# rcallahan/smalt

Hardware: AMD Instinct MI355X
Metric: mapped reads/sec (1Mx150bp vs 3Gbp ref) (higher is better)
Workload: dtype f16

## Files before the change

### smalt_amd/csrc/smg_kernels.hip

```cpp
#include <hip/hip_runtime.h>
#include <cstdlib>
#include "smg_kernels.h"
#include "smg_stages.hpp"

namespace smg {

__device__ inline uint8_t code_of(uint8_t c) {
  c &= 0xDF;
  return c == 'A' ? 0 : c == 'C' ? 1 : c == 'G' ? 2 : (c == 'T' || c == 'U') ? 3 : 5;
}

__global__ void __launch_bounds__(64) k_encode(const uint8_t *bases, const uint64_t *off, uint32_t n, uint8_t *codes, uint8_t *codes_rc) {
  for (uint32_t r = blockIdx.x; r < n; r += gridDim.x) {
    const uint64_t o = off[r];
    const uint32_t len = (uint32_t)(off[r + 1] - o);
    for (uint32_t i = threadIdx.x; i < len; i += 64) {
      uint8_t c = code_of(bases[o + i]);
      codes[o + i] = c;
      codes_rc[o + len - 1 - i] = (c & 4) ? c : (uint8_t)(3 - c);
    }
  }
}

__global__ void __launch_bounds__(64) k_gather_reads(uint8_t *dst_bases, uint8_t *dst_quals, const uint64_t *dst_off, uint32_t n, const uint32_t *ids,
// ... 171 lines not shown
  __shared__ uint32_t qslot;
  uint32_t *cursor = b.next_item + NEXT_ITEM_STRIDE * (pass == 2 ? 3 : 2);
  if (pass == 2) {
    const uint32_t n = *b.align_retry_n;
    for (uint32_t i = next_item(cursor, &qslot); i < n; i = next_item(cursor, &qslot)) {
      stage_align<WIDE>(b, ix, p, b.align_retry[i], x);
      __syncthreads();
    }
    align_tally_flush(b, x);
    return;
  }
  for (uint32_t r = next_item(cursor, &qslot); r < b.nreads; r = next_item(cursor, &qslot)) {
    stage_align<WIDE>(b, ix, p, r, x);
    __syncthreads();
  }
  align_tally_flush(b, x);
}

template <int G>
__device__ inline int shr1(int v) {
  return __builtin_amdgcn_update_dpp(0, v, 0x111 , 0xf, 0xf, true);
}

template <int G, int C>
__global__ void __launch_bounds__(64) k_sw_full(Batch b, DevIndex ix, MapPar p, uint32_t ntask_cap, int after16) {
  if (after16 && b.work[WK_QN_TASKS] == 0) return;
  constexpr int NG = 64 / G;
  constexpr int WMAX = SW_FULL_WMAX;
  __shared__ uint8_t win[NG][WMAX + 8];
  __shared__ uint2 tab[8];
  const int lane = threadIdx.x, g = lane % G, grp = lane / G;
  const uint32_t ntask = min(*b.rc_count, ntask_cap);
  const int bias = (p.mismatch < p.mismatch - p.match ? -p.mismatch : -(p.mismatch - p.match));
  const int gi = -p.gap_init, ge = -p.gap_ext;
  if (lane < 8) {
    int rb = lane == 7 ? 0 : ((lane == 6 || lane == 4) ? 5 : lane);
    uint32_t w[2] = {0, 0};
    for (int qc = 0; qc < 8; qc++) {
      int v = (rb == 5 || qc >= 4) ? 0 : ((rb == qc) ? p.match : p.mismatch);
      w[qc >> 2] |= (uint32_t)((v + bias) & 0xff) << (8 * (qc & 3));
    }
    tab[lane] = make_uint2(w[0], w[1]);
  }
  __syncthreads();
  const uint32_t ngroups = gridDim.x * NG;
  unsigned long long cells = 0, ntasks_done = 0;
  for (uint32_t t0 = blockIdx.x * NG; t0 < ntask; t0 += ngroups) {
    const uint32_t t = t0 + grp;
    RCand c;
    bool live = false;
    uint32_t qlen = 0, wlen = 0;
    uint64_t gbase = 0;
    if (t < ntask) {
      c = b.rcpool[t];
      qlen = read_len(b, c.rid);
      wlen = (uint32_t)(c.re - c.rs + 1);
      live = !(c.flags & (RCF_BANDED | RCF_ERR | RCF_SCORED)) && wlen <= (uint32_t)WMAX && qlen <= (uint32_t)(G * C);
      gbase = (c.sqidx < 0 ? 0ull : ix.sop[c.sqidx]) + c.rs;
    }
    if (!live) { qlen = 0; wlen = 0; }
    for (uint32_t i = g; i < wlen; i += G) win[grp][i] = (uint8_t)ref_code(ix.packed, gbase + i);
    uint32_t sel[C];
    {
      const uint8_t *q = ((c.flags & RCF_REVERSE) ? b.codes_rc : b.codes) + (live ? b.read_off[c.rid] : 0);
#pragma unroll
      for (int cc = 0; cc < C; cc++) {
        uint32_t j = (uint32_t)(g * C + cc);
        uint32_t qc = (live && j < qlen) ? q[j] : 5u;
        sel[cc] = 0x0c0c0c00u | qc;
      }
    }
    int H[C], E[C];
#pragma unroll
    for (int cc = 0; cc < C; cc++) { H[cc] = 0; E[cc] = 0; }
    int best = 0, F = 0, prev_hl = 0;
    int nstep = (int)wlen + G - 1;
    for (int o = 32; o > 0; o >>= 1) nstep = max(nstep, __shfl_xor(nstep, o));
    __syncthreads();
    for (int step = 0; step < nstep; step++) {
      const int row = step - g;
      const uint32_t rb = (row >= 0 && row < (int)wlen) ? win[grp][row] : 5u;
      const uint2 tr = tab[rb];
      int hl = shr1<G>(H[C - 1]);
      int fin = shr1<G>(F);
      if (g == 0) { hl = 0; fin = 0; }
      int diag = prev_hl;
      prev_hl = hl;
      F = fin;
#pragma unroll
      for (int cc = 0; cc < C; cc++) {
        const int w = (int)__builtin_amdgcn_perm(tr.y, tr.x, sel[cc]);
        const int h = diag + w - bias;
        const int hh = max(max(h, E[cc]), F);
        best = max(best, hh);
        diag = H[cc];
        H[cc] = hh;
        const int tt = hh - gi;
        E[cc] = max(max(E[cc] - ge, tt), 0);
        F = max(max(F - ge, tt), 0);
      }
    }
    for (int o = G / 2; o > 0; o >>= 1) best = max(best, __shfl_xor(best, o));
    if (live && g == 0) {
      b.rcpool[t].swscor = best;
      b.rcpool[t].flags = c.flags | RCF_SCORED | (best >= 65535 ? RCF_BANDED : 0u);
      cells += (unsigned long long)qlen * wlen;
      ntasks_done += best < 65535 ? 1 : 0;
    }
    __syncthreads();
  }
  for (int o = 32; o > 0; o >>= 1) { cells += __shfl_xor(cells, o); ntasks_done += __shfl_xor(ntasks_done, o); }
  if (lane == 0 && cells) { atomicAdd(b.work + WK_CELLS_FULL, cells); atomicAdd(b.work + WK_TASKS_FULL, ntasks_done); }
}

typedef unsigned short us2 __attribute__((ext_vector_type(2)));
__device__ inline us2 as_us2(uint32_t v) { return __builtin_bit_cast(us2, v); }
__device__ inline uint32_t as_u32(us2 v) { return __builtin_bit_cast(uint32_t, v); }
__device__ inline us2 pk_max(us2 a, us2 b) { return __builtin_elementwise_max(a, b); }
__device__ inline us2 pk_subs(us2 a, us2 b) { return __builtin_elementwise_sub_sat(a, b); }
__device__ inline us2 pk_add_nc(us2 a, us2 b) { return as_us2(as_u32(a) + as_u32(b)); }
typedef _Float16 hf2 __attribute__((ext_vector_type(2)));
__device__ inline us2 pk_max3(us2 a, us2 b, us2 c) {
  const hf2 r = __builtin_elementwise_maximum(__builtin_elementwise_maximum(__builtin_bit_cast(hf2, a), __builtin_bit_cast(hf2, b)), __builtin_bit_cast(hf2, c));
  return __builtin_bit_cast(us2, r);
}
__device__ inline uint32_t shr1_u32(uint32_t v) { return (uint32_t)__builtin_amdgcn_update_dpp(0, (int)v, 0x111 , 0xf, 0xf, true); }

enum : int { SW16_BLK = 5 };
struct Sw16Par { uint32_t mm4, dlt, n4; us2 bias, gi, ge; int fp; uint32_t hi_match, hi_mismatch; us2 ngi, nge; };
__device__ inline uint32_t f16_bits_of_int(int n) {
  if (n == 0) return 0;
  const uint32_t sign = n < 0 ? 0x8000u : 0u, a = (uint32_t)(n < 0 ? -n : n);
  const int e = 31 - __clz((int)a);
  return sign | ((uint32_t)(e + 15) << 10) | ((e <= 10 ? a << (10 - e) : a >> (e - 10)) & 0x3ffu);
}
__device__ inline Sw16Par sw16_par(const MapPar &p, int ncols = 512) {
  Sw16Par s;
  const uint32_t fm = f16_bits_of_int(p.match), fx = f16_bits_of_int(p.mismatch);
  s.fp = (fm & 0xffu) == 0 && (fx & 0xffu) == 0 && p.match > 0 && p.match * ncols <= 2040 && -p.gap_init >= 0 && -p.gap_init <= 2040 &&
         -p.gap_ext >= 0 && -p.gap_ext <= 2040 && p.mismatch >= -1024;
  s.hi_match = fm >> 8; s.hi_mismatch = fx >> 8;
  { const uint32_t a = f16_bits_of_int(p.gap_init), e = f16_bits_of_int(p.gap_ext);
    s.ngi = us2{(unsigned short)a, (unsigned short)a}; s.nge = us2{(unsigned short)e, (unsigned short)e}; }
  const int bias = (p.mismatch < p.mismatch - p.match ? -p.mismatch : -(p.mismatch - p.match));
  s.mm4 = (uint32_t)((p.mismatch + bias) & 0xff) * 0x01010101u;
  s.dlt = (uint32_t)(p.match - p.mismatch);
  s.n4 = (uint32_t)(bias & 0xff) * 0x01010101u;
  s.bias = us2{(unsigned short)bias, (unsigned short)bias};
  s.gi = us2{(unsigned short)(-p.gap_init), (unsigned short)(-p.gap_init)};
  s.ge = us2{(unsigned short)(-p.gap_ext), (unsigned short)(-p.gap_ext)};
  return s;
}

template <int G, int C>
__device__ inline uint32_t sw16_core(const uint16_t *wrow, int nstep, const uint32_t (&sel)[C], int g, const Sw16Par &sp, const uint2 *rowtab2) {
  us2 H[C], E[C];
#pragma unroll
  for (int cc = 0; cc < C; cc++) { H[cc] = us2{0, 0}; E[cc] = us2{0, 0}; }
  us2 best = us2{0, 0}, F = us2{0, 0}, prev_hl = us2{0, 0};
  const uint32_t gmask = g == 0 ? 0u : 0xffffffffu;
  for (int step = 0; step < nstep; step++) {
    const uint2 rr = rowtab2[wrow[step - g + (G - 1)]];
    const uint32_t rowA = rr.x, rowB = rr.y;
    const uint32_t hl = shr1_u32(as_u32(H[C - 1])) & gmask;
    const uint32_t fin = shr1_u32(as_u32(F)) & gmask;
    us2 carry = prev_hl;
    prev_hl = as_us2(hl);
    F = as_us2(fin);
#pragma unroll
    for (int c0 = 0; c0 < C; c0 += SW16_BLK) {
      us2 t3[SW16_BLK];
      const us2 last_old = H[(c0 + SW16_BLK - 1 < C) ? c0 + SW16_BLK - 1 : C - 1];
#pragma unroll
      for (int u = 0; u < SW16_BLK; u++) {
        const int cc = c0 + u;
        if (cc < C) {
          const us2 w = as_us2(__builtin_amdgcn_perm(rowB, rowA, sel[cc]));
          const us2 dg = u == 0 ? carry : H[cc - 1];
          t3[u] = pk_subs(pk_add_nc(dg, w), sp.bias);
        }
      }
#pragma unroll
      for (int u = 0; u < SW16_BLK; u++) {
        const int cc = c0 + u;
        if (cc < C) {
          const us2 hh = pk_max3(t3[u], E[cc], F);
          H[cc] = hh;
          const us2 tt = pk_subs(hh, sp.gi);
          E[cc] = pk_max(pk_subs(E[cc], sp.ge), tt);
          F = pk_max(pk_subs(F, sp.ge), tt);
        }
      }
#pragma unroll
      for (int u = 0; u < SW16_BLK; u += 2) {
        const int cc = c0 + u;
        if (cc + 1 < C && u + 1 < SW16_BLK) best = pk_max3(best, H[cc], H[cc + 1]);
        else if (cc < C) best = pk_max(best, H[cc]);
      }
      carry = last_old;
    }
  }
  uint32_t bb = as_u32(best);
  for (int o = G / 2; o > 0; o >>= 1) bb = as_u32(pk_max(as_us2(bb), as_us2((uint32_t)__shfl_xor((int)bb, o))));
  return bb;
}

__device__ inline hf2 hf_max3(hf2 a, hf2 b, hf2 c) { return __builtin_elementwise_maximum(__builtin_elementwise_maximum(a, b), c); }
template <int G, int C>
__device__ inline uint32_t sw16f_core(const uint16_t *wrow, int nstep, const uint32_t (&sel)[C], int g, const Sw16Par &sp, const uint2 *rowtab2) {
  hf2 H[C], E[C];
  const hf2 zero = hf2{(_Float16)0, (_Float16)0};
#pragma unroll
  for (int cc = 0; cc < C; cc++) { H[cc] = zero; E[cc] = zero; }
  hf2 best = zero, F = zero, prev_hl = zero;
  const hf2 ngi = __builtin_bit_cast(hf2, sp.ngi), nge = __builtin_bit_cast(hf2, sp.nge);
  const uint32_t gmask = g == 0 ? 0u : 0xffffffffu;
  for (int step = 0; step < nstep; step++) {
    const uint2 rr = rowtab2[wrow[step - g + (G - 1)]];
    const uint32_t hl = shr1_u32(__builtin_bit_cast(uint32_t, H[C - 1])) & gmask;
    const uint32_t fin = shr1_u32(__builtin_bit_cast(uint32_t, F)) & gmask;
    hf2 carry = prev_hl;
    prev_hl = __builtin_bit_cast(hf2, hl);
    F = __builtin_bit_cast(hf2, fin);
#pragma unroll
    for (int c0 = 0; c0 < C; c0 += SW16_BLK) {
      hf2 t3[SW16_BLK];
      const hf2 last_old = H[(c0 + SW16_BLK - 1 < C) ? c0 + SW16_BLK - 1 : C - 1];
#pragma unroll
      for (int u = 0; u < SW16_BLK; u++) {
        const int cc = c0 + u;
        if (cc < C) {
          const hf2 w = __builtin_bit_cast(hf2, __builtin_amdgcn_perm(rr.y, rr.x, sel[cc]));
          const hf2 dg = u == 0 ? carry : H[cc - 1];
          t3[u] = dg + w;
        }
      }
#pragma unroll
      for (int u = 0; u < SW16_BLK; u++) {
        const int cc = c0 + u;
        if (cc < C) {
          const hf2 hh = hf_max3(t3[u], E[cc], F);
          H[cc] = hh;
          const hf2 tt = hh + ngi;
          E[cc] = hf_max3(E[cc] + nge, tt, zero);
          F = hf_max3(F + nge, tt, zero);
        }
      }
#pragma unroll
      for (int u = 0; u < SW16_BLK; u += 2) {
        const int cc = c0 + u;
        if (cc + 1 < C && u + 1 < SW16_BLK) best = hf_max3(best, H[cc], H[cc + 1]);
        else if (cc < C) best = __builtin_elementwise_maximum(best, H[cc]);
      }
      carry = last_old;
    }
  }
  for (int o = G / 2; o > 0; o >>= 1)
    best = __builtin_elementwise_maximum(best, __builtin_bit_cast(hf2, (uint32_t)__shfl_xor((int)__builtin_bit_cast(uint32_t, best), o)));
  return (uint32_t)(int)(float)best.x | ((uint32_t)(int)(float)best.y << 16);
}

__device__ inline void sw16_rowtab(uint32_t *rowtab, const Sw16Par &sp) {
  if (threadIdx.x < 8) rowtab[threadIdx.x] = threadIdx.x < 4 ? sp.mm4 + (sp.dlt << (8 * threadIdx.x)) : sp.n4;
}
__device__ inline void sw16_rowtab2(uint2 *rowtab2, const Sw16Par &sp) {
  const uint32_t a = threadIdx.x & 7u, bq = threadIdx.x >> 3;
  if (sp.fp) {
    const uint32_t x4 = sp.hi_mismatch * 0x01010101u;
    rowtab2[threadIdx.x] = make_uint2(a < 4 ? (x4 & ~(0xffu << (8 * a))) | (sp.hi_match << (8 * a)) : 0u,
                                      bq < 4 ? (x4 & ~(0xffu << (8 * bq))) | (sp.hi_match << (8 * bq)) : 0u);
    return;
  }
  rowtab2[threadIdx.x] = make_uint2(a < 4 ? sp.mm4 + (sp.dlt << (8 * a)) : sp.n4, bq < 4 ? sp.mm4 + (sp.dlt << (8 * bq)) : sp.n4);
}
enum : uint32_t { SW16_NPAIR = 5u | (5u << 3) };

template <int G, int C, int WMAX>
__global__ void __launch_bounds__(64) k_sw_full16(Batch b, DevIndex ix, MapPar p, uint32_t ntask_cap) {
  const unsigned long long nlong = WMAX > SW_SHORT_WMAX ? b.work[WK_LONG_TASKS] : 0;
  if (WMAX > SW_SHORT_WMAX && nlong == 0) return;
  const uint32_t *list = (WMAX > SW_SHORT_WMAX && b.long_list && nlong <= b.long_cap) ? b.long_list : nullptr;
  constexpr int NG = 64 / G;
  __shared__ uint16_t win[NG][WMAX + 2 * G];
  __shared__ uint2 rowtab2[64];
  const int lane = threadIdx.x, g = lane % G, grp = lane / G;
  const uint32_t ntask = list ? (uint32_t)nlong : min(*b.rc_count, ntask_cap), npair = (ntask + 1) / 2;
  const Sw16Par sp = sw16_par(p, G * C);
  sw16_rowtab2(rowtab2, sp);
  const uint32_t ngroups = gridDim.x * NG;
  unsigned long long cells = 0, ntasks_done = 0;
  for (uint32_t t0 = blockIdx.x * NG; t0 < npair; t0 += ngroups) {
    const uint32_t tp = t0 + grp;
    RCand c[2];
    bool live[2] = {false, false};
    uint32_t qlen[2] = {0, 0}, wlen[2] = {0, 0}, tix[2] = {0, 0};
    uint64_t gbase[2] = {0, 0};
    const uint8_t *q[2] = {b.codes, b.codes};
#pragma unroll
    for (int u = 0; u < 2; u++) {
      const uint32_t tl = 2 * tp + (uint32_t)u;
      if (tp < npair && tl < ntask) {
        tix[u] = list ? list[tl] : tl;
        c[u] = b.rcpool[tix[u]];
        qlen[u] = read_len(b, c[u].rid);
        wlen[u] = (uint32_t)(c[u].re - c[u].rs + 1);
        live[u] = !(c[u].flags & (RCF_BANDED | RCF_ERR | RCF_QN | RCF_SCORED)) && wlen[u] <= (uint32_t)WMAX && qlen[u] <= (uint32_t)(G * C);
        gbase[u] = (c[u].sqidx < 0 ? 0ull : ix.sop[c[u].sqidx]) + c[u].rs;
        q[u] = ((c[u].flags & RCF_REVERSE) ? b.codes_rc : b.codes) + b.read_off[c[u].rid];
      }
      if (!live[u]) { qlen[u] = 0; wlen[u] = 0; }
    }
    const uint32_t wmax = wlen[0] > wlen[1] ? wlen[0] : wlen[1];
    int nstep = (int)wmax + G - 1;
    for (int o = 32; o > 0; o >>= 1) nstep = max(nstep, __shfl_xor(nstep, o));
    nstep = __builtin_amdgcn_readfirstlane(nstep);
    {
      const uint32_t nent = (uint32_t)(nstep + G - 1), per = (nent + G - 1) / G;
      const uint32_t e0 = (uint32_t)g * per, e1 = e0 + per < nent ? e0 + per : nent;
      const uint64_t lastw = ix.totlen / 10;
      uint64_t wi[2] = {0, 0};
      uint32_t wd[2] = {0, 0}, nx[2] = {0, 0}, off[2] = {0, 0};
#pragma unroll
      for (int u = 0; u < 2; u++) {
        const int i0 = (int)e0 - (G - 1);
        const uint64_t pos = gbase[u] + (uint64_t)(i0 > 0 ? i0 : 0);
        wi[u] = pos / 10; off[u] = (uint32_t)(pos - wi[u] * 10);
        if (wlen[u] && e0 < e1) { wd[u] = ix.packed[wi[u] < lastw ? wi[u] : lastw]; nx[u] = ix.packed[wi[u] + 1 < lastw ? wi[u] + 1 : lastw]; }
      }
      for (uint32_t e = e0; e < e1; e++) {
        const uint32_t i = e - (uint32_t)(G - 1);
        uint32_t cd[2];
#pragma unroll
        for (int u = 0; u < 2; u++) {
          cd[u] = 5u;
          if (i < wlen[u]) {
            const uint32_t c = (wd[u] >> (3 * (9 - off[u]))) & 7u;
            cd[u] = (c == 7) ? 0u : ((c == 6 || c == 4) ? 5u : c);
            if (++off[u] == 10) { off[u] = 0; wi[u]++; wd[u] = nx[u]; nx[u] = ix.packed[wi[u] + 1 < lastw ? wi[u] + 1 : lastw]; }
          }
        }
        win[grp][e] = (uint16_t)(cd[0] | (cd[1] << 3));
      }
    }
    uint32_t sel[C];
#pragma unroll
    for (int cc = 0; cc < C; cc++) {
      const uint32_t j = (uint32_t)(g * C + cc);
      const uint32_t sa = j < qlen[0] ? (uint32_t)q[0][j] : 0x0cu, sb = j < qlen[1] ? 4u + (uint32_t)q[1][j] : 0x0cu;
      sel[cc] = sp.fp ? (0x000c000cu | (sa << 8) | (sb << 24)) : (0x0c000c00u | sa | (sb << 16));
    }
    __syncthreads();
    const uint32_t bb = sp.fp ? sw16f_core<G, C>(win[grp], nstep, sel, g, sp, rowtab2) : sw16_core<G, C>(win[grp], nstep, sel, g, sp, rowtab2);
    if (g == 0) {
#pragma unroll
      for (int u = 0; u < 2; u++) {
        if (live[u]) {
          const int best = (int)((bb >> (16 * u)) & 0xffffu);
          const uint32_t t = tix[u];
          b.rcpool[t].swscor = best;
          b.rcpool[t].flags = c[u].flags | RCF_SCORED | (best >= 65535 ? RCF_BANDED : 0u);
          cells += (unsigned long long)qlen[u] * wlen[u];
          ntasks_done += best < 65535 ? 1 : 0;
        }
      }
    }
    __syncthreads();
  }
  for (int o = 32; o > 0; o >>= 1) { cells += __shfl_xor(cells, o); ntasks_done += __shfl_xor(ntasks_done, o); }
  if (lane == 0 && cells) { atomicAdd(b.work + WK_CELLS_FULL, cells); atomicAdd(b.work + WK_TASKS_FULL, ntasks_done); }
}

template <int G, int C>
__global__ void __launch_bounds__(64) k_sw_full16_raw(const uint8_t *qcodes, const uint32_t *q_off, const uint8_t *rcodes,
                                                       const uint32_t *r_off, uint32_t ntask, MapPar p, int32_t *scores) {
  constexpr int NG = 64 / G;
  constexpr int WMAX = SW_FULL_WMAX;
  __shared__ uint16_t win[NG][WMAX + 2 * G];
  __shared__ uint2 rowtab2[64];
  const int lane = threadIdx.x, g = lane % G, grp = lane / G;
  const uint32_t npair = (ntask + 1) / 2;
  const Sw16Par sp = sw16_par(p, G * C);
  sw16_rowtab2(rowtab2, sp);
  const uint32_t ngroups = gridDim.x * NG;
  for (uint32_t t0 = blockIdx.x * NG; t0 < npair; t0 += ngroups) {
    const uint32_t tp = t0 + grp;
    bool live[2] = {false, false};
    uint32_t qlen[2] = {0, 0}, wlen[2] = {0, 0};
    const uint8_t *q[2] = {qcodes, qcodes}, *r[2] = {rcodes, rcodes};
#pragma unroll
    for (int u = 0; u < 2; u++) {
      const uint32_t t = 2 * tp + (uint32_t)u;
      if (tp < npair && t < ntask) {
        qlen[u] = q_off[t + 1] - q_off[t]; wlen[u] = r_off[t + 1] - r_off[t];
        q[u] += q_off[t]; r[u] += r_off[t];
        live[u] = wlen[u] <= (uint32_t)WMAX && qlen[u] <= (uint32_t)(G * C);
      }
      if (!live[u]) { qlen[u] = 0; wlen[u] = 0; }
    }
    const uint32_t wmax = wlen[0] > wlen[1] ? wlen[0] : wlen[1];
    int nstep = (int)wmax + G - 1;
    for (int o = 32; o > 0; o >>= 1) nstep = max(nstep, __shfl_xor(nstep, o));
    nstep = __builtin_amdgcn_readfirstlane(nstep);
    for (uint32_t e = g; e < (uint32_t)(nstep + G - 1); e += G) {
      const uint32_t i = e - (uint32_t)(G - 1);
      uint32_t cd[2];
#pragma unroll
      for (int u = 0; u < 2; u++) { const uint32_t x = i < wlen[u] ? (r[u][i] & 7u) : 5u; cd[u] = x == 7 ? 0 : ((x == 6 || x == 4) ? 5 : x); }
      win[grp][e] = (uint16_t)(cd[0] | (cd[1] << 3));
    }
    uint32_t sel[C];
    bool qn[2] = {false, false};
#pragma unroll
    for (int cc = 0; cc < C; cc++) {
      const uint32_t j = (uint32_t)(g * C + cc);
      uint32_t s2[2];
#pragma unroll
      for (int u = 0; u < 2; u++) {
        const uint32_t qc = j < qlen[u] ? (q[u][j] & 7u) : 0x0cu;
        if (j < qlen[u] && qc >= 4) qn[u] = true;
        s2[u] = qc == 0x0cu ? 0x0cu : (uint32_t)(4 * u) + (qc & 3u);
      }
      sel[cc] = sp.fp ? (0x000c000cu | (s2[0] << 8) | (s2[1] << 24)) : (0x0c000c00u | s2[0] | (s2[1] << 16));
    }
#pragma unroll
    for (int u = 0; u < 2; u++) for (int o = G / 2; o > 0; o >>= 1) { const int other = __shfl_xor((int)qn[u], o); qn[u] = qn[u] || other != 0; }
    __syncthreads();
    const uint32_t bb = sp.fp ? sw16f_core<G, C>(win[grp], nstep, sel, g, sp, rowtab2) : sw16_core<G, C>(win[grp], nstep, sel, g, sp, rowtab2);
    if (g == 0) {
#pragma unroll
      for (int u = 0; u < 2; u++) {
        const uint32_t t = 2 * tp + (uint32_t)u;
        if (tp < npair && t < ntask) scores[t] = !live[u] ? -1 : (qn[u] ? -2 : (int)((bb >> (16 * u)) & 0xffffu));
      }
    }
    __syncthreads();
  }
}

enum : int { SW_STRIP_C = 16 };

__device__ inline int sw_strip_core(const uint8_t *q, uint32_t qlen, const uint8_t *win, uint32_t wlen, int2 *bnd, uint32_t wcap,
                                    const uint2 *tab, int2 *ring , int bias, int gi, int ge) {
  constexpr int C = SW_STRIP_C;
  const int g = (int)threadIdx.x;
  int2 *ring_in = ring, *ring_out = ring + 128;
  int best = 0;
  const uint32_t nstrip = (qlen + 64 * C - 1) / (64 * C);
  const int nstep = (int)wlen + 63;
  for (uint32_t sidx = 0; sidx < nstrip; sidx++) {
    const int2 *bprev = bnd + (size_t)((sidx + 1) & 1) * wcap;
    int2 *bnext = bnd + (size_t)(sidx & 1) * wcap;
    uint32_t sel[C];
#pragma unroll
    for (int cc = 0; cc < C; cc++) {
      const uint32_t j = sidx * 64 * C + (uint32_t)(g * C + cc);
      sel[cc] = 0x0c0c0c00u | (j < qlen ? (uint32_t)(q[j] & 7) : 5u);
    }
    int H[C], E[C];
#pragma unroll
    for (int cc = 0; cc < C; cc++) { H[cc] = 0; E[cc] = 0; }
    int F = 0, prev_hl = 0;
    __syncthreads();
    if (sidx > 0) {
      const int r0 = g;
      ring_in[g] = r0 < (int)wlen ? bprev[r0] : make_int2(0, 0);
    }
    __syncthreads();
    for (int step = 0; step < nstep; step++) {
      const int row = step - g;
      if (sidx > 0 && (step & 63) == 0) {
        const int r1 = step + 64 + g;
        ring_in[((step >> 6) + 1) % 2 * 64 + g] = r1 < (int)wlen ? bprev[r1] : make_int2(0, 0);
      }
      const uint32_t rb = (row >= 0 && row < (int)wlen) ? win[row] : 5u;
      const uint2 tr = tab[rb];
      int hl = wave_shr1(H[C - 1]);
      int fin = wave_shr1(F);
      if (g == 0) {
        if (sidx > 0) { const int2 v = ring_in[(step >> 6) % 2 * 64 + (step & 63)]; hl = step < (int)wlen ? v.x : 0; fin = step < (int)wlen ? v.y : 0; }
        else { hl = 0; fin = 0; }
      }
      int diag = prev_hl;
      prev_hl = hl;
      F = fin;
#pragma unroll
      for (int cc = 0; cc < C; cc++) {
        const int w = (int)__builtin_amdgcn_perm(tr.y, tr.x, sel[cc]);
        const int h = diag + w - bias;
        const int hh = max(max(h, E[cc]), F);
        best = max(best, hh);
        diag = H[cc];
        H[cc] = hh;
        const int tt = hh - gi;
        E[cc] = max(max(E[cc] - ge, tt), 0);
        F = max(max(F - ge, tt), 0);
      }
      if (sidx + 1 < nstrip) {
        if (g == 63 && row >= 0 && row < (int)wlen) ring_out[row & 127] = make_int2(H[C - 1], F);
        const int rdone = step - 63;
        if (rdone >= 0 && ((rdone & 63) == 63 || rdone == (int)wlen - 1)) {
          __syncthreads();
          const int base = rdone & ~63, r2 = base + g;
          if (r2 <= rdone && r2 < (int)wlen) bnext[r2] = ring_out[r2 & 127];
        }
      }
      if (sidx > 0 && (step & 63) == 63) __syncthreads();
    }
    __threadfence();
  }
  for (int o = 32; o > 0; o >>= 1) best = max(best, __shfl_xor(best, o));
  return best;
}

__device__ inline void sw_tab8(uint2 *tab, const MapPar &p, int bias) {
  if (threadIdx.x < 8) {
    const int lane = (int)threadIdx.x;
    const int rb = lane == 7 ? 0 : ((lane == 6 || lane == 4) ? 5 : lane);
    uint32_t w[2] = {0, 0};
    for (int qc = 0; qc < 8; qc++) {
      const int v = (rb == 5 || qc >= 4) ? 0 : ((rb == qc) ? p.match : p.mismatch);
      w[qc >> 2] |= (uint32_t)((v + bias) & 0xff) << (8 * (qc & 3));
    }
    tab[lane] = make_uint2(w[0], w[1]);
  }
}

template <bool M3>
__device__ inline uint32_t sw_strip16_core(const uint8_t *qa, uint32_t qlen_a, const uint8_t *qb, uint32_t qlen_b, const uint16_t *win2, uint32_t wmax,
                                           uint2 *bnd, uint32_t wcap, const uint32_t *rowtab, uint2 *ring , const Sw16Par &sp) {
  constexpr int C = SW_STRIP_C;
  const int g = (int)threadIdx.x;
  uint2 *ring_in = ring, *ring_out = ring + 128;
  us2 best = us2{0, 0};
  const uint32_t qmaxlen = qlen_a > qlen_b ? qlen_a : qlen_b;
  const uint32_t nstrip = (qmaxlen + 64 * C - 1) / (64 * C);
  const int nstep = (int)wmax + 63;
  for (uint32_t sidx = 0; sidx < nstrip; sidx++) {
    const uint2 *bprev = bnd + (size_t)((sidx + 1) & 1) * wcap;
    uint2 *bnext = bnd + (size_t)(sidx & 1) * wcap;
    uint32_t sel[C];
#pragma unroll
    for (int cc = 0; cc < C; cc++) {
      const uint32_t j = sidx * 64 * C + (uint32_t)(g * C + cc);
      const uint32_t sa = j < qlen_a ? (uint32_t)(qa[j] & 3) : 0x0cu, sb = j < qlen_b ? 4u + (uint32_t)(qb[j] & 3) : 0x0cu;
      sel[cc] = 0x0c000c00u | sa | (sb << 16);
    }
    us2 H[C], E[C];
#pragma unroll
    for (int cc = 0; cc < C; cc++) { H[cc] = us2{0, 0}; E[cc] = us2{0, 0}; }
    us2 F = us2{0, 0}, prev_hl = us2{0, 0};
    __syncthreads();
    if (sidx > 0) ring_in[g] = g < (int)wmax ? bprev[g] : make_uint2(0, 0);
    __syncthreads();
    for (int step = 0; step < nstep; step++) {
      const int row = step - g;
      if (sidx > 0 && (step & 63) == 0) {
        const int r1 = step + 64 + g;
        ring_in[((step >> 6) + 1) % 2 * 64 + g] = r1 < (int)wmax ? bprev[r1] : make_uint2(0, 0);
      }
      const uint32_t rp = (row >= 0 && row < (int)wmax) ? win2[row] : 0x0505u;
      const uint32_t rowA = rowtab[rp & 0xffu], rowB = rowtab[rp >> 8];
// ... 599 lines not shown
```

### smalt_amd/csrc/smg_logic.hpp

```cpp
#pragma once
#include "smg_common.h"

namespace smg {

template <class T> SMG_HD inline T tmin(T a, T b) { return a < b ? a : b; }
template <class T> SMG_HD inline T tmax(T a, T b) { return a > b ? a : b; }

SMG_HD inline uint32_t hash32mix(uint32_t a) {
  a = (a + 0x7ed55d16u) + (a << 12);
  a = (a ^ 0xc761c23cu) ^ (a >> 19);
  a = (a + 0x165667b1u) + (a << 5);
  a = (a + 0xd3a2646cu) ^ (a << 9);
  a = (a + 0xfd7046c5u) + (a << 3);
  a = (a ^ 0xb55a4f09u) ^ (a >> 16);
  return a;
}

SMG_HD inline uint32_t index_lookup(const DevIndex &ix, uint64_t word, uint32_t *posidx) {
  const uint64_t wordmask = (1ull << (2 * ix.k)) - 1;
  if (ix.typ == IDX_PERFECT) {
    uint32_t key = (uint32_t)(word & wordmask);
    *posidx = key;
    return ix.idx[key + 1] - ix.idx[key];
  }
  const uint64_t mask_lo = (1ull << ix.nbits_lo) - 1;
  const uint32_t keymod = 1u << (ix.nbits_key - ix.nbits_lo);
  uint32_t word_hi = (uint32_t)((word & wordmask & ~mask_lo) >> ix.nbits_lo);
  uint32_t key = ((hash32mix(word_hi) % keymod) << ix.nbits_lo) + (uint32_t)(word & mask_lo);
  uint32_t b = ix.idx[key + 1];
  if (b < 1) return 0;
  uint32_t a = ix.idx[key];
  b--;
  while (a < b) {
    uint32_t pivot = (a + b) >> 1;
    if (ix.wordidx[pivot] < word_hi) a = pivot + 1; else b = pivot;
  }
  if (a == b && ix.wordidx[b] == word_hi) {
    *posidx = b;
    return ix.posidx[b + 1] - ix.posidx[b];
  }
  return 0;
}

SMG_HD inline uint32_t index_positions(const DevIndex &ix, uint32_t posidx, const uint32_t **posp) {
  if (ix.typ == IDX_PERFECT) {
    *posp = ix.pos + ix.idx[posidx];
    return ix.idx[posidx + 1] - ix.idx[posidx];
  }
  *posp = ix.pos + ix.posidx[posidx];
  return ix.posidx[posidx + 1] - ix.posidx[posidx];
}

SMG_HD inline uint32_t ref_code(const uint32_t *packed, uint64_t o) {
  uint32_t w = packed[o / 10];
  uint32_t c = (w >> (3 * (9 - (uint32_t)(o % 10)))) & 7u;
  return (c == 7) ? 0u : ((c == 6 || c == 4) ? 5u : c);
}

SMG_HD inline void sort2_u32(int n, uint32_t *key, uint32_t *val) {
  int lo = 0, hi = n - 1, i, j, mid, sp = 0;
  int stk[64];
  uint32_t pk, pv, t;
#define SMG_SWP(a, b) { t = key[a]; key[a] = key[b]; key[b] = t; t = val[a]; val[a] = val[b]; val[b] = t; }
  for (;;) {
    if (hi - lo < 7) {
      for (j = lo + 1; j <= hi; j++) {
        pk = key[j]; pv = val[j];
        for (i = j - 1; i >= lo && key[i] > pk; i--) { key[i + 1] = key[i]; val[i + 1] = val[i]; }
        key[i + 1] = pk; val[i + 1] = pv;
      }
      if (!sp) return;
      hi = stk[sp--]; lo = stk[sp--];
    } else {
      mid = (lo + hi) >> 1;
      SMG_SWP(mid, lo + 1)
      if (key[lo] > key[hi]) SMG_SWP(lo, hi)
      if (key[lo + 1] > key[hi]) SMG_SWP(lo + 1, hi)
      if (key[lo] > key[lo + 1]) SMG_SWP(lo, lo + 1)
      i = lo + 1; j = hi;
      pk = key[lo + 1]; pv = val[lo + 1];
      for (;;) {
        do i++; while (key[i] < pk);
        do j--; while (key[j] > pk);
        if (j < i) break;
        SMG_SWP(i, j)
      }
      key[lo + 1] = key[j]; key[j] = pk;
      val[lo + 1] = val[j]; val[j] = pv;
      sp += 2;
      if (sp > 60) return;
      if (hi - i + 1 >= j - lo) { stk[sp] = hi; stk[sp - 1] = i; hi = j - 1; }
      else { stk[sp] = j - 1; stk[sp - 1] = lo; lo = i; }
    }
  }
#undef SMG_SWP
}

SMG_HD inline void build_frames(uint32_t n_seeds, const uint32_t *qoffs_by_rank, int s, uint32_t *frame_cnt,
                                uint32_t *frame_rank, uint32_t stride) {
  for (int f = 0; f < s; f++) frame_cnt[f] = 0;
  for (uint32_t i = 0; i < n_seeds; i++) {
    uint32_t f = qoffs_by_rank[i] % (uint32_t)s;
    frame_rank[f * stride + frame_cnt[f]++] = i;
  }
}

SMG_HD inline uint32_t seed_max_rank(uint32_t n_seeds, const uint32_t *sortkey, const uint32_t *qoffs_by_rank, int k, int s,
                                     uint32_t qlen, uint32_t mincover, uint32_t maxcover, uint32_t maxhit,
                                     const uint32_t *frame_cnt, const uint32_t *frame_rank, uint32_t stride, uint8_t *qbuf) {
  uint32_t i, ntot = sortkey[0];
  for (i = 1; i <= n_seeds && ntot <= maxhit; i++)
    if (i < n_seeds) ntot += sortkey[i];
  uint32_t n = i - 1, nmax = n;
  for (int f = 0; f < s; f++) {
    uint32_t imax = frame_cnt[f];
    if (!imax) continue;
    const uint32_t *ixp = frame_rank + (uint32_t)f * stride;
    for (uint32_t q = 0; q < qlen; q++) qbuf[q] = 0;
    uint32_t cover = 0;
    for (i = 0; i < imax && cover <= maxcover && (cover < mincover || ixp[i] <= n); i++) {
      uint32_t q0 = qoffs_by_rank[ixp[i]];
      for (uint32_t q = q0; q < q0 + (uint32_t)k - 1; q++)
        if (!qbuf[q]) { qbuf[q] = 1; cover++; }
    }
    if (i > 0 && ixp[i - 1] > nmax) nmax = ixp[i - 1];
  }
  if (nmax < (uint32_t)HITINFO_MINSEEDNUM) return ((uint32_t)HITINFO_MINSEEDNUM < n_seeds) ? (uint32_t)HITINFO_MINSEEDNUM : n_seeds;
  return nmax;
}

SMG_HD inline uint32_t cover_deficit(uint32_t status, uint32_t seed_rank, uint32_t qlen, const uint8_t *qmask,
                                     const uint32_t *qoffs_by_rank, int k, int s, const uint32_t *frame_cnt,
                                     const uint32_t *frame_rank, uint32_t stride, uint8_t *qbuf) {
  uint32_t deficit, d, i;
  if (status & HI_RANK) {
    uint32_t maxcover = 0;
    d = qlen;
    for (int f = 0; f < s; f++) {
      uint32_t imax = frame_cnt[f];
      if (!imax) continue;
      const uint32_t *ixp = frame_rank + (uint32_t)f * stride;
      for (uint32_t q = 0; q < qlen; q++) qbuf[q] = 0;
      uint32_t cover = 0;
      for (i = 0; i < imax && ixp[i] < seed_rank; i++) {
        uint32_t q0 = qoffs_by_rank[ixp[i]];
        for (uint32_t q = q0; q < q0 + (uint32_t)k; q++)
          if (!qbuf[q]) { qbuf[q] = 1; cover++; }
      }
      if (cover < d) d = cover;
      if (cover > maxcover) maxcover = cover;
    }
    deficit = maxcover - d + 1;
  } else {
    uint8_t kk = (uint8_t)(k / s);
    if (kk > 0) kk--;
    deficit = 0;
    for (int f = 0; f < s; f++) {
      uint8_t ctr = 0;
      d = 0;
      for (i = (uint32_t)f; i < qlen; i += (uint32_t)s) {
        if (qmask[i] == HQ_NORMHIT) ctr = kk;
        else if (ctr) ctr--;
        else d += (uint32_t)s;
      }
      if (d > deficit) deficit = d;
    }
  }
  return deficit;
}

SMG_HD inline uint64_t hit_diag(bool is_reverse, uint32_t pos, uint32_t q, int s) {
  const uint64_t offbit = 1ull << 32;
  return is_reverse ? ((uint64_t)pos + q / (uint32_t)s) : ((((uint64_t)pos) | offbit) - q / (uint32_t)s);
}

SMG_HD inline uint32_t div_magic(int s) { return s > 1 ? (uint32_t)((0x100000000ull + (uint32_t)s - 1) / (uint32_t)s) : 0u; }
SMG_HD inline uint64_t hit_diag_m(bool is_reverse, uint32_t pos, uint32_t q, uint32_t magic) {
  const uint64_t offbit = 1ull << 32;
  const uint32_t qs = magic ? (uint32_t)(((uint64_t)q * magic) >> 32) : q;
  return is_reverse ? ((uint64_t)pos + qs) : ((((uint64_t)pos) | offbit) - qs);
}

SMG_HD inline uint32_t lower_bound_u32(const uint32_t *a, uint32_t n, uint32_t v) {
  uint32_t lo = 0, hi = n;
  while (lo < hi) { uint32_t m = (lo + hi) >> 1; if (a[m] < v) lo = m + 1; else hi = m; }
  return lo;
}

SMG_HD inline void lower_bounds2_u32(const uint32_t *a, uint32_t n, uint32_t lo, uint32_t hi, uint32_t *at_lo, uint32_t *at_hi) {
  if (n <= 32) {
    uint32_t below_lo = 0, below_hi = 0;
    for (uint32_t j0 = 0; j0 < n; j0 += 16) {
      uint32_t v[16];
#pragma unroll
      for (uint32_t u = 0; u < 16; u++) v[u] = j0 + u < n ? a[j0 + u] : 0xffffffffu;
#pragma unroll
      for (uint32_t u = 0; u < 16; u++) { below_lo += v[u] < lo ? 1u : 0u; below_hi += v[u] < hi ? 1u : 0u; }
    }
    *at_lo = below_lo; *at_hi = below_hi;
    return;
  }
  *at_lo = lower_bound_u32(a, n, lo);
  *at_hi = *at_lo + lower_bound_u32(a + *at_lo, n - *at_lo, hi);
}

struct FillDecision { uint32_t n_used; uint32_t m_final; };

SMG_HD inline FillDecision fill_decide(const DevIndex &ix, const SeedRec *seeds, uint32_t n_seeds, uint32_t lo, uint32_t hi,
                                       uint32_t nhit_max, int nhits_alloc, uint8_t *qmask) {
// ... 433 lines not shown
```

Baseline: 771,700.

## Vectorize SW16 window and query staging, unroll DP loop by two

The window of reference codes is now built ten bases at a time. Each step reads two packed words and decodes them with bitwise SWAR mapping, then writes 32-bit pairs to shared memory, replacing the old per-base sequential decode. Query selectors are built from aligned dword loads with alignbyte and perm instead of byte loads. Row-table entries are pre-shifted so a byte offset can be used directly, the f16 DP loop is unrolled by two with nstep rounded to even, and the wave-wide max uses DPP and readlane. The added complexity risks subtle boundary errors in the window clipping and in the padded extra step.

```diff
diff --git a/smalt_amd/csrc/smg_kernels.hip b/smalt_amd/csrc/smg_kernels.hip
--- a/smalt_amd/csrc/smg_kernels.hip
+++ b/smalt_amd/csrc/smg_kernels.hip
@@ -347,6 +347,7 @@
   return s;
 }
 
+__device__ inline uint2 sw16_row(const uint2 *rowtab2, uint32_t entry) { return *(const uint2 *)((const char *)rowtab2 + entry); }
 template <int G, int C>
 __device__ inline uint32_t sw16_core(const uint16_t *wrow, int nstep, const uint32_t (&sel)[C], int g, const Sw16Par &sp, const uint2 *rowtab2) {
   us2 H[C], E[C];
@@ -355,7 +356,7 @@
   us2 best = us2{0, 0}, F = us2{0, 0}, prev_hl = us2{0, 0};
   const uint32_t gmask = g == 0 ? 0u : 0xffffffffu;
   for (int step = 0; step < nstep; step++) {
-    const uint2 rr = rowtab2[wrow[step - g + (G - 1)]];
+    const uint2 rr = sw16_row(rowtab2, wrow[step - g + (G - 1)]);
     const uint32_t rowA = rr.x, rowB = rr.y;
     const uint32_t hl = shr1_u32(as_u32(H[C - 1])) & gmask;
     const uint32_t fin = shr1_u32(as_u32(F)) & gmask;
@@ -410,8 +411,8 @@
   hf2 best = zero, F = zero, prev_hl = zero;
   const hf2 ngi = __builtin_bit_cast(hf2, sp.ngi), nge = __builtin_bit_cast(hf2, sp.nge);
   const uint32_t gmask = g == 0 ? 0u : 0xffffffffu;
-  for (int step = 0; step < nstep; step++) {
-    const uint2 rr = rowtab2[wrow[step - g + (G - 1)]];
+  auto row = [&](int step) __attribute__((always_inline)) {
+    const uint2 rr = sw16_row(rowtab2, wrow[step - g + (G - 1)]);
     const uint32_t hl = shr1_u32(__builtin_bit_cast(uint32_t, H[C - 1])) & gmask;
     const uint32_t fin = shr1_u32(__builtin_bit_cast(uint32_t, F)) & gmask;
     hf2 carry = prev_hl;
@@ -449,7 +450,8 @@
       }
       carry = last_old;
     }
-  }
+  };
+  for (int step = 0; step < nstep; step += 2) { row(step); row(step + 1); }
   for (int o = G / 2; o > 0; o >>= 1)
     best = __builtin_elementwise_maximum(best, __builtin_bit_cast(hf2, (uint32_t)__shfl_xor((int)__builtin_bit_cast(uint32_t, best), o)));
   return (uint32_t)(int)(float)best.x | ((uint32_t)(int)(float)best.y << 16);
@@ -468,7 +470,19 @@
   }
   rowtab2[threadIdx.x] = make_uint2(a < 4 ? sp.mm4 + (sp.dlt << (8 * a)) : sp.n4, bq < 4 ? sp.mm4 + (sp.dlt << (8 * bq)) : sp.n4);
 }
-enum : uint32_t { SW16_NPAIR = 5u | (5u << 3) };
+enum : uint32_t { SW16_NPAIR = 5u | (5u << 3), SW16_ESHIFT = 3  };
+
+typedef uint32_t __attribute__((may_alias)) u32a;
+
+template <int G>
+__device__ inline int wave_max_groups(int v) {
+  static_assert(G == 4 || G == 8 || G == 16, "the row folds below cover groups of 4, 8 or 16 lanes");
+  if (G <= 4) v = max(v, __builtin_amdgcn_update_dpp(v, v, 0x124 , 0xf, 0xf, false));
+  if (G <= 8) v = max(v, __builtin_amdgcn_update_dpp(v, v, 0x128 , 0xf, 0xf, false));
+  return max(max(__builtin_amdgcn_readlane(v, 0), __builtin_amdgcn_readlane(v, 16)), max(__builtin_amdgcn_readlane(v, 32), __builtin_amdgcn_readlane(v, 48)));
+}
+
+constexpr int sw16_wrow(int G, int WMAX) { return (WMAX + 2 * G + 9) / 10 * 10; }
 
 template <int G, int C, int WMAX>
 __global__ void __launch_bounds__(64) k_sw_full16(Batch b, DevIndex ix, MapPar p, uint32_t ntask_cap) {
@@ -476,16 +490,25 @@
   if (WMAX > SW_SHORT_WMAX && nlong == 0) return;
   const uint32_t *list = (WMAX > SW_SHORT_WMAX && b.long_list && nlong <= b.long_cap) ? b.long_list : nullptr;
   constexpr int NG = 64 / G;
-  __shared__ uint16_t win[NG][WMAX + 2 * G];
+  constexpr int WROW = sw16_wrow(G, WMAX);
+  __shared__ uint32_t win32[NG][WROW / 2];
   __shared__ uint2 rowtab2[64];
   const int lane = threadIdx.x, g = lane % G, grp = lane / G;
+  const uint16_t *wrow = (const uint16_t *)win32[grp];
   const uint32_t ntask = list ? (uint32_t)nlong : min(*b.rc_count, ntask_cap), npair = (ntask + 1) / 2;
   const Sw16Par sp = sw16_par(p, G * C);
   sw16_rowtab2(rowtab2, sp);
   const uint32_t ngroups = gridDim.x * NG;
+  const uint64_t lastw = ix.totlen / 10;
+  const uint32_t sel_or = sp.fp ? 0x000c000cu : 0x0c000c00u;
+  uint32_t sel_pick[4];
+#pragma unroll
+  for (uint32_t i = 0; i < 4; i++) sel_pick[i] = sp.fp ? (0x000c000cu | (i << 8) | ((4u + i) << 24)) : (0x0c000c00u | i | ((4u + i) << 16));
   unsigned long long cells = 0, ntasks_done = 0;
   for (uint32_t t0 = blockIdx.x * NG; t0 < npair; t0 += ngroups) {
     const uint32_t tp = t0 + grp;
+    int gs = g;
+    asm volatile("" : "+v"(gs));
     RCand c[2];
     bool live[2] = {false, false};
     uint32_t qlen[2] = {0, 0}, wlen[2] = {0, 0}, tix[2] = {0, 0};
@@ -503,49 +526,69 @@
         gbase[u] = (c[u].sqidx < 0 ? 0ull : ix.sop[c[u].sqidx]) + c[u].rs;
         q[u] = ((c[u].flags & RCF_REVERSE) ? b.codes_rc : b.codes) + b.read_off[c[u].rid];
       }
-      if (!live[u]) { qlen[u] = 0; wlen[u] = 0; }
+      if (!live[u]) { qlen[u] = 0; wlen[u] = 0; gbase[u] = 0; q[u] = b.codes; }
     }
     const uint32_t wmax = wlen[0] > wlen[1] ? wlen[0] : wlen[1];
-    int nstep = (int)wmax + G - 1;
-    for (int o = 32; o > 0; o >>= 1) nstep = max(nstep, __shfl_xor(nstep, o));
-    nstep = __builtin_amdgcn_readfirstlane(nstep);
+    const int nstep = (wave_max_groups<G>((int)wmax + G - 1) + 1) & ~1;
     {
-      const uint32_t nent = (uint32_t)(nstep + G - 1), per = (nent + G - 1) / G;
-      const uint32_t e0 = (uint32_t)g * per, e1 = e0 + per < nent ? e0 + per : nent;
-      const uint64_t lastw = ix.totlen / 10;
-      uint64_t wi[2] = {0, 0};
-      uint32_t wd[2] = {0, 0}, nx[2] = {0, 0}, off[2] = {0, 0};
+      const int nblk = (nstep + G - 1 + 9) / 10;
+      const uint32_t *pw[2];
+      uint32_t o0[2];
+      int relmax[2];
 #pragma unroll
       for (int u = 0; u < 2; u++) {
-        const int i0 = (int)e0 - (G - 1);
-        const uint64_t pos = gbase[u] + (uint64_t)(i0 > 0 ? i0 : 0);
-        wi[u] = pos / 10; off[u] = (uint32_t)(pos - wi[u] * 10);
-        if (wlen[u] && e0 < e1) { wd[u] = ix.packed[wi[u] < lastw ? wi[u] : lastw]; nx[u] = ix.packed[wi[u] + 1 < lastw ? wi[u] + 1 : lastw]; }
-      }
-      for (uint32_t e = e0; e < e1; e++) {
-        const uint32_t i = e - (uint32_t)(G - 1);
-        uint32_t cd[2];
+        uint64_t w = gbase[u] / 10;
+        o0[u] = (uint32_t)(gbase[u] - w * 10);
+        if (w > lastw) w = lastw;
+        const uint64_t left = lastw - w;
+        relmax[u] = left < 4096 ? (int)left : 4096;
+        pw[u] = ix.packed + w;
+      }
+      for (int kb = 0; kb < nblk; kb += G) {
+        const int k = kb + gs, i0 = 10 * k - (G - 1);
+        uint32_t y[2];
 #pragma unroll
         for (int u = 0; u < 2; u++) {
-          cd[u] = 5u;
-          if (i < wlen[u]) {
-            const uint32_t c = (wd[u] >> (3 * (9 - off[u]))) & 7u;
-            cd[u] = (c == 7) ? 0u : ((c == 6 || c == 4) ? 5u : c);
-            if (++off[u] == 10) { off[u] = 0; wi[u]++; wd[u] = nx[u]; nx[u] = ix.packed[wi[u] + 1 < lastw ? wi[u] + 1 : lastw]; }
+          static_assert(G <= 16, "win_block10 takes first rows down to -20");
+          y[u] = win_block10(pw[u], o0[u], relmax[u], i0, wlen[u]);
+        }
+        if (k < nblk) {
+          u32a *dst = (u32a *)&win32[grp][5 * k];
+#pragma unroll
+          for (int j = 0; j < 5; j++) {
+            const uint32_t s0 = 3u * (9u - 2u * j), s1 = s0 - 3u;
+            const uint32_t ea = ((y[0] >> s0) & 7u) | (((y[1] >> s0) & 7u) << 3), eb = ((y[0] >> s1) & 7u) | (((y[1] >> s1) & 7u) << 3);
+            dst[j] = (ea | (eb << 16)) << SW16_ESHIFT;
           }
         }
-        win[grp][e] = (uint16_t)(cd[0] | (cd[1] << 3));
       }
     }
     uint32_t sel[C];
-#pragma unroll
-    for (int cc = 0; cc < C; cc++) {
-      const uint32_t j = (uint32_t)(g * C + cc);
-      const uint32_t sa = j < qlen[0] ? (uint32_t)q[0][j] : 0x0cu, sb = j < qlen[1] ? 4u + (uint32_t)q[1][j] : 0x0cu;
-      sel[cc] = sp.fp ? (0x000c000cu | (sa << 8) | (sb << 24)) : (0x0c000c00u | sa | (sb << 16));
-    }
-    __syncthreads();
-    const uint32_t bb = sp.fp ? sw16f_core<G, C>(win[grp], nstep, sel, g, sp, rowtab2) : sw16_core<G, C>(win[grp], nstep, sel, g, sp, rowtab2);
+    {
+      constexpr int ND = (C + 3) / 4;
+      uint32_t qd[2][ND];
+#pragma unroll
+      for (int u = 0; u < 2; u++) {
+        const uint32_t mis = (uint32_t)(uintptr_t)q[u] & 3u;
+        const u32a *q4 = (const u32a *)(q[u] - mis);
+        const uint32_t b0 = mis + (uint32_t)(gs * C), d0 = b0 >> 2;
+        const uint32_t lastd = (mis + (qlen[u] ? qlen[u] - 1 : 0u)) >> 2;
+        uint32_t raw[ND + 1];
+#pragma unroll
+        for (int k = 0; k <= ND; k++) raw[k] = q4[min(d0 + (uint32_t)k, lastd)];
+#pragma unroll
+        for (int k = 0; k < ND; k++) {
+          const uint32_t d = __builtin_amdgcn_alignbyte(raw[k + 1], raw[k], b0 & 3u) + (u ? 0x04040404u : 0u);
+          const int nv = min(max((int)qlen[u] - (gs * C + 4 * k), 0), 4);
+          const uint32_t m = nv >= 4 ? 0xffffffffu : (1u << (8 * nv)) - 1u;
+          qd[u][k] = (d & m) | (0x0c0c0c0cu & ~m);
+        }
+      }
+#pragma unroll
+      for (int cc = 0; cc < C; cc++) sel[cc] = __builtin_amdgcn_perm(qd[1][cc / 4], qd[0][cc / 4], sel_pick[cc & 3]) | sel_or;
+    }
+    __syncthreads();
+    const uint32_t bb = sp.fp ? sw16f_core<G, C>(wrow, nstep, sel, g, sp, rowtab2) : sw16_core<G, C>(wrow, nstep, sel, g, sp, rowtab2);
     if (g == 0) {
 #pragma unroll
       for (int u = 0; u < 2; u++) {
@@ -595,13 +638,13 @@
     const uint32_t wmax = wlen[0] > wlen[1] ? wlen[0] : wlen[1];
     int nstep = (int)wmax + G - 1;
     for (int o = 32; o > 0; o >>= 1) nstep = max(nstep, __shfl_xor(nstep, o));
-    nstep = __builtin_amdgcn_readfirstlane(nstep);
+    nstep = (__builtin_amdgcn_readfirstlane(nstep) + 1) & ~1;
     for (uint32_t e = g; e < (uint32_t)(nstep + G - 1); e += G) {
       const uint32_t i = e - (uint32_t)(G - 1);
       uint32_t cd[2];
 #pragma unroll
       for (int u = 0; u < 2; u++) { const uint32_t x = i < wlen[u] ? (r[u][i] & 7u) : 5u; cd[u] = x == 7 ? 0 : ((x == 6 || x == 4) ? 5 : x); }
-      win[grp][e] = (uint16_t)(cd[0] | (cd[1] << 3));
+      win[grp][e] = (uint16_t)((cd[0] | (cd[1] << 3)) << SW16_ESHIFT);
     }
     uint32_t sel[C];
     bool qn[2] = {false, false};
diff --git a/smalt_amd/csrc/smg_logic.hpp b/smalt_amd/csrc/smg_logic.hpp
--- a/smalt_amd/csrc/smg_logic.hpp
+++ b/smalt_amd/csrc/smg_logic.hpp
@@ -55,6 +55,31 @@
   uint32_t w = packed[o / 10];
   uint32_t c = (w >> (3 * (9 - (uint32_t)(o % 10)))) & 7u;
   return (c == 7) ? 0u : ((c == 6 || c == 4) ? 5u : c);
+}
+
+SMG_HD inline uint32_t win_codes10(uint32_t w0, uint32_t w1, uint32_t off) {
+  const uint64_t v = ((uint64_t)(w0 & 0x3fffffffu) << 30) | (uint64_t)(w1 & 0x3fffffffu);
+  return (uint32_t)(v >> (3u * (10u - off))) & 0x3fffffffu;
+}
+enum : uint32_t { WIN_BIT2 = 0x24924924u , WIN_N10 = 0x2db6db6du  };
+SMG_HD inline uint32_t win_map10(uint32_t x) {
+  const uint32_t b2 = x & WIN_BIT2, is7 = b2 & (x << 1) & (x << 2), isn = b2 & ~is7;
+  const uint32_t ge4 = b2 | (b2 >> 1) | (b2 >> 2);
+  return (x & ~ge4) | isn | (isn >> 2);
+}
+SMG_HD inline uint32_t win_clip10(uint32_t x, int lo, int hi) {
+  const uint32_t m = ((1u << (3 * (hi - lo))) - 1u) << (3 * (10 - hi));
+  return (x & m) | (WIN_N10 & ~m);
+}
+
+SMG_HD inline uint32_t win_block10(const uint32_t *pw, uint32_t o0, int relmax, int i0, uint32_t wlen) {
+  const uint32_t t = (uint32_t)((int)o0 + i0 + 20);
+  const uint32_t tq = t / 10u, off = t - 10u * tq;
+  const int wq = (int)tq - 2, wa = wq < 0 ? 0 : wq, wb = wq + 1 < 0 ? 0 : wq + 1;
+  const uint32_t w0 = pw[wa < relmax ? wa : relmax], w1 = pw[wb < relmax ? wb : relmax];
+  const int l = -i0, h = (int)wlen - i0;
+  const int lo = l < 0 ? 0 : (l > 10 ? 10 : l), hi = h < 0 ? 0 : (h > 10 ? 10 : h);
+  return win_clip10(win_map10(win_codes10(w0, w1, off)), lo, hi);
 }
 
 SMG_HD inline void sort2_u32(int n, uint32_t *key, uint32_t *val) {
```

New measurement: 807,500 (median of 6 runs). +4.6%, better.
